# walaj/SeqLib

Hardware: AMD Instinct MI355X
Metric: aligned reads/sec (150 bp) via BWAAligner (higher is better)
Workload: dtype int32

## Files before the change

seqlib_amd/csrc/dev_chain.h:

```cpp
#pragma once
#include "dev_fm.h"
#include "dev_sort.h"
#include "dev_types.h"
#include "dev_pack.h"
#include "dev_kbtree.h"

__device__ __forceinline__ int next_slot(unsigned int *queue, int per_wave = 0)
{
    const int lane = threadIdx.x & 63;
    const unsigned int base = wave_take(queue, per_wave ? 1u : 64u);
    if (per_wave) return lane == 0 ? (int)base : 0x7fffffff;
    return (int)(base + lane);
}

struct ReadWS {
    int64_t *s_rbeg; qp_t *s_ql; int32_t *s_next; int32_t *s_score;
    int64_t *c_pos; int32_t *c_head, *c_tail, *c_n, *c_rid, *c_w, *c_first; int8_t *c_kept;
    int32_t *ia, *ib, *ic; uint64_t *srt;
    DReg *regs; DHit *hits;
    int cap;
    __device__ __forceinline__ int s_qbeg(int s) const { return QP_HI(s_ql[s]); }
    __device__ __forceinline__ int s_len(int s) const { return QP_LO(s_ql[s]); }
};

// ... 32 lines not shown
    for (int s = w.c_head[c]; s >= 0; s = w.s_next[s]) {
        const int qb = w.s_qbeg(s), l = w.s_len(s);
        if (qb >= end) wt += l;
        else if (qb + l > end) wt += (int)(qb + l - end);
        end = end > qb + l ? end : qb + l;
    }
    tmp = wt; wt = 0; end = 0;
    for (int s = w.c_head[c]; s >= 0; s = w.s_next[s]) {
        const int64_t rb = w.s_rbeg[s]; const int l = w.s_len(s);
        if (rb >= end) wt += l;
        else if (rb + l > end) wt += (int)(rb + l - end);
        end = end > rb + l ? end : rb + l;
    }
    wt = wt < tmp ? wt : tmp;
    return wt < 1 << 30 ? wt : (1 << 30) - 1;
}

template <typename I>
__device__ void dev_chain_read(const DevFM<I> &fm, const DevRef &R, const Chunk &ck, const slx_opt &opt, int r)
{
        ReadWS w = make_ws(ck, r);
        const int len = (int)(ck.offs[r + 1] - ck.offs[r]);
        const int n_intv = (int)ck.intv_n[r];
        const qp_t *iinfo = (const qp_t *)ck.intv_info + (size_t)r * ck.cap_intv;
        const I *ix0 = (const I *)ck.intv_x0 + (size_t)r * ck.cap_intv;
        const I *ix2 = (const I *)ck.intv_x2 + (size_t)r * ck.cap_intv;
        int ns = 0, nc = 0;
        int *ord = w.ia;
        KbTree kb;
        bool tree = false;
        int cc = -1, cc_tail = 0, cc_n = 0, cc_rid = 0;
        qp_t cc_fql = 0, cc_lql = 0;
        int64_t cc_frb = 0, cc_lrb = 0;
        for (int i = 0; i < n_intv; ++i) {
            const int qbeg = QP_HI(iinfo[i]), slen = QP_LO(iinfo[i]) - qbeg;
            const I x2 = ix2[i];
            const I step = x2 > (I)opt.max_occ ? x2 / (I)opt.max_occ : (I)1;
            I k = 0;
            for (int count = 0; k < x2 && count < opt.max_occ; k += step, ++count) {
                const int64_t rbeg = intv_pos<I>(fm, ix0[i], k);
                const int rid = dev_intv2rid(R, rbeg, rbeg + slen);
                if (rid < 0) continue;
                int lo = -1, lower_c = -1;
                bool to_add = true;
                if (nc) {
                    if (tree) lower_c = kb.lower(rbeg);
                    else {
                        int b = 0, e = nc;
                        while (b < e) { int m = (b + e) >> 1; if (w.c_pos[ord[m]] < rbeg) b = m + 1; else e = m; }
                        if (b == nc) lo = nc - 1;
                        else lo = rbeg < w.c_pos[ord[b]] ? b - 1 : b;
                        lower_c = lo >= 0 ? ord[lo] : -1;
                    }
                    if (lower_c >= 0) {
                        const int c = lower_c;
                        if (c != cc) {
                            const int first = w.c_head[c];
                            cc = c; cc_tail = w.c_tail[c]; cc_n = w.c_n[c]; cc_rid = w.c_rid[c];
                            cc_fql = w.s_ql[first]; cc_frb = w.s_rbeg[first];
                            cc_lql = w.s_ql[cc_tail]; cc_lrb = w.s_rbeg[cc_tail];
                        }
                        const int last = cc_tail;
                        const int l_qbeg = QP_HI(cc_lql), l_len = QP_LO(cc_lql);
                        const int64_t l_rbeg = cc_lrb;
                        const int64_t qend = l_qbeg + l_len, rend = l_rbeg + l_len;
                        int res;
                        if (rid != cc_rid) res = 0;
                        else if (qbeg >= QP_HI(cc_fql) && qbeg + slen <= qend && rbeg >= cc_frb && rbeg + slen <= rend) res = 1;
                        else if ((l_rbeg < R.l_pac || cc_frb < R.l_pac) && rbeg >= R.l_pac) res = 0;
                        else {
                            const int64_t x = qbeg - l_qbeg, y = rbeg - l_rbeg;
                            if (y >= 0 && x - y <= opt.w && y - x <= opt.w && x - l_len < opt.max_chain_gap && y - l_len < opt.max_chain_gap) {
                                const int s = ns++;
// ... 77 lines not shown
            int s_full = -1, cov = 0;
            bool same_diag = true;
            int64_t diag = 0;
            for (int s = w.c_head[c0]; s >= 0; s = w.s_next[s])
                if (w.s_qbeg(s) == 0 && w.s_len(s) == len) { s_full = s; diag = w.s_rbeg[s]; break; }
            if (s_full >= 0) {
                for (int s = w.c_head[c0]; s >= 0; s = w.s_next[s]) {
                    cov += w.s_len(s);
                    if (w.s_rbeg[s] - w.s_qbeg(s) != diag) same_diag = false;
                }
                if (same_diag) {
                    DReg g;
                    g.rb = diag; g.re = g.rb + len; g.qb = 0; g.qe = len; g.rid = w.c_rid[c0];
                    g.score = g.truesc = len * opt.a; g.sub = g.csub = g.sub_n = 0; g.w = opt.w; g.seedcov = cov; g.secondary = 0;
                    g.seedlen0 = len; g.n_comp = 0; g.frac_rep = ck.frac_rep[r]; g.hash = 0;
                    w.regs[0] = g;
                    ck.n_reg[r] = 1;
                    n_out = -1;
                }
            }
        }
        {
            int off = 0;
            for (int i = 0; i < n_out; ++i) {
                const int c = a[i];
                w.c_first[c] = off;
                for (int s = w.c_head[c]; s >= 0; s = w.s_next[s]) w.c_w[off++] = s;
            }
        }
        ck.n_chain[r] = n_out;
}

template <typename I>
__global__ void __launch_bounds__(128) k_chain(DevFM<I> fm, DevRef R, Chunk ck, DevOpt dopt, const int *order, unsigned int *queue, const unsigned int *n_slots, int per_wave)
{
    const slx_opt &opt = dopt.o;
    const int n_todo = (int)*n_slots;
    if (per_wave) __builtin_amdgcn_s_setprio(3);
    while (true) {
        const int slot = next_slot(queue, per_wave);
        if (__all(slot >= n_todo)) break;
        if (slot >= n_todo) continue;
        const int r = order ? order[slot] : slot;
        dev_chain_read<I>(fm, R, ck, opt, r);
    }
}
```

seqlib_amd/csrc/dev_fm.h:

```cpp
#pragma once
#include <hip/hip_runtime.h>
#include <stdint.h>

template <typename I>
struct DevFM {
    const uint32_t *bwt;
    const uint4 *occ;
    const uint64_t *sup;
    I primary;
    I L2[5];
    I seq_len;
    const I *sa_dense;
    const uint64_t *sa_samp;
    int sa_intv;
    const void *lut;
    int lut_k;
    int bwd_direct;
    const uint32_t *rep;
    uint64_t rep_mask;
    int rep_k;
};

__host__ __device__ __forceinline__ uint64_t rep_hash(uint64_t kmer)
{
    kmer ^= kmer >> 33; kmer *= 0xff51afd7ed558ccdull; kmer ^= kmer >> 33; kmer *= 0xc4ceb9fe1a85ec53ull; kmer ^= kmer >> 33;
    return kmer;
}

template <typename I>
struct alignas(2 * sizeof(I)) LutE { I lo, sz; };

template <typename I>
struct alignas(16) IntvE {
    I x0, x1, x2;
    uint32_t info;
};

template <typename I>
struct WorkLists {
    IntvE<I> *base;
    size_t stride;
    int cap;
    __device__ __forceinline__ IntvE<I> &at(int list, int e) { return base[((size_t)list * cap + e) * stride]; }
};

__device__ __forceinline__ void count_word(uint32_t w, int nb, uint32_t &c, uint32_t &g, uint32_t &t)
{
    uint32_t mask = nb >= 16 ? 0xffffffffu : (nb <= 0 ? 0u : ~(0xffffffffu >> (2 * nb)));
    w &= mask;
    uint32_t lo = w & 0x55555555u, hi = (w >> 1) & 0x55555555u;
    t += __popc(hi & lo);
    g += __popc(hi & ~lo);
    c += __popc(lo & ~hi);
// ... 98 lines not shown
```

seqlib_amd/csrc/dev_seed4.h:

```cpp
#pragma once
#include "dev_occ.h"
#include "dev_pack.h"

template <typename I>
struct RankLd {
    uint32_t c0, c1, c2, c3;
    uint32_t l0, l1, h0, h1;
    I s0, s1, s2, s3;
    uint32_t n;
};

template <typename I>
__device__ __forceinline__ void rank_issue(const DevFM<I> &fm, I pos, RankLd<I> &r)
{
    const I kk = pos - (pos >= fm.primary ? 1 : 0);
    const uint4 *blk = fm.occ + ((size_t)(kk >> 6) << 1);
    const uint4 cn = blk[0], pl = blk[1];
    r.c0 = cn.x; r.c1 = cn.y; r.c2 = cn.z; r.c3 = cn.w;
    r.l0 = pl.x; r.l1 = pl.y; r.h0 = pl.z; r.h1 = pl.w;
    r.n = ((uint32_t)kk & 63) + 1;
    if (sizeof(I) == 8) {
        const ulonglong2 *sp = (const ulonglong2 *)(fm.sup + ((uint64_t)kk >> 32) * 4);
        const ulonglong2 a = sp[0], b = sp[1];
        r.s0 = (I)a.x; r.s1 = (I)a.y; r.s2 = (I)b.x; r.s3 = (I)b.y;
    } else r.s0 = r.s1 = r.s2 = r.s3 = 0;
}

template <typename T>
__device__ __forceinline__ T sel4(int c, T v0, T v1, T v2, T v3) { const T lo = (c & 1) ? v1 : v0, hi = (c & 1) ? v3 : v2; return (c & 2) ? hi : lo; }

template <typename I, bool GT>
__device__ __forceinline__ void rank_finish(const RankLd<I> &r, int c, I &cnt_c, I &cnt_gt)
{
    const uint64_t m = ~0ull >> (64 - r.n);
    const uint32_t m0 = (uint32_t)m, m1 = (uint32_t)(m >> 32);
// ... 76 lines not shown
}

template <typename I>
__device__ __forceinline__ void fwd_step(const DevFM<I> &fm, I k0, I k1, I k2, int cq, I &o0, I &o1, I &o2)
{
    const int c = 3 - cq;
    RankLd<I> rk, rl;
    rank_issue<I>(fm, k1 - 1, rk); rank_issue<I>(fm, k1 - 1 + k2, rl);
    I ckc, ckg, clc, clg;
    rank_finish<I, true>(rk, c, ckc, ckg); rank_finish<I, true>(rl, c, clc, clg);
    o2 = clc - ckc;
    o1 = l2_of<I>(fm, c) + 1 + ckc;
    o0 = k0 + ((k1 <= fm.primary && k1 + k2 - 1 >= fm.primary) ? 1 : 0) + (clg - ckg);
}

template <typename I>
__global__ void k_kmer_lut(DevFM<I> fm, int K, LutE<I> *out)
{
    const uint64_t w = (uint64_t)blockIdx.x * blockDim.x + threadIdx.x;
    if (w >= (1ull << (2 * K))) return;
    I k0, k1, k2;
    set_intv4<I>(fm, (int)((w >> (2 * (K - 1))) & 3), k0, k1, k2);
    for (int t = 1; t < K; ++t) {
        I o0, o1, o2;
        fwd_step<I>(fm, k0, k1, k2, (int)((w >> (2 * (K - 1 - t))) & 3), o0, o1, o2);
        k0 = o0; k1 = o1; k2 = o2;
        if (k2 == 0) break;
    }
    LutE<I> e; e.lo = k2 ? k0 : (I)1; e.sz = k2;
    out[w] = e;
}

template <typename I>
__global__ void k_rep_filter(DevFM<I> fm, DevRef R, int kf, uint32_t *bits, uint64_t mask)
{
    const uint64_t n = (uint64_t)fm.seq_len;
    const uint64_t stride = (uint64_t)gridDim.x * blockDim.x;
    for (uint64_t i = (uint64_t)blockIdx.x * blockDim.x + threadIdx.x; i < n; i += stride) {
        const uint64_t p = (uint64_t)fm.sa_dense[i], q = (uint64_t)fm.sa_dense[i + 1];
        if (p + (uint64_t)kf > n || q + (uint64_t)kf > n) continue;
        RWin wp, wq; wp.bits = wq.bits = 0; wp.chunk = wq.chunk = -1;
        uint64_t kmer = 0;
        bool same = true;
        for (int t = 0; t < kf; ++t) {
            const int a = text_at(R, (int64_t)(p + t), wp), b = text_at(R, (int64_t)(q + t), wq);
            if (a != b) { same = false; break; }
            kmer = (kmer << 2) | (uint64_t)a;
        }
        if (!same) continue;
        const uint64_t h = rep_hash(kmer) & mask;
        atomicOr(bits + (h >> 5), 1u << (h & 31));
    }
}

template <typename I>
__global__ void __launch_bounds__(128) k_seed2_select(DevFM<I> fm, Chunk ck, DevOpt dopt, unsigned long long *p2mask, int *list, unsigned int *n_list,
                                                      uint32_t *items, unsigned int *n_items, uint32_t cap_items)
{
    const slx_opt &opt = dopt.o;
    const int t_ = blockIdx.x * blockDim.x + threadIdx.x;
    const int r = ck.spread > 1 ? t_ / ck.spread : t_;
    const bool live = r < ck.n_reads && (ck.spread <= 1 || t_ % ck.spread == 0);
    const int n = live ? (int)ck.intv_n[r] : 0;
    unsigned long long mask = 0;
    if (n > 0) {
        const uint64_t qoff = ck.offs[r];
        const int len = (int)(ck.offs[r + 1] - qoff);
        const int split_len = (int)(opt.min_seed_len * opt.split_factor + .499);
        QWin win; win.bits = 0; win.chunk = 0xffffffffu;
        auto qb = [&](int p) { return q_at(ck.codes, qoff + (uint64_t)p, win); };
        const bool use_rep = fm.rep != nullptr && fm.rep_k <= opt.min_seed_len && fm.rep_k > 0;
        const int kf = fm.rep_k;
        const uint64_t kmask = kf < 32 ? (1ull << (2 * kf)) - 1 : ~0ull;
        for (int k = 0; k < n; ++k) {
            const size_t o = (size_t)r * ck.cap_intv + k;
            const qp_t inf = ((const qp_t *)ck.intv_info)[o];
            const I s = ((const I *)ck.intv_x2)[o];
            const int start = QP_HI(inf), end = QP_LO(inf);
            if (end - start < split_len || s > (I)opt.split_width) continue;
            if (k >= 63) { mask |= 1ull << 63; break; }
            const int mid = (start + end) >> 1;
            if (qb(mid) > 3) continue;
            bool take = true;
            if (s == (I)1 && use_rep) {
                const int a_lo = mid - kf + 1 > 0 ? mid - kf + 1 : 0, a_hi = mid < len - kf ? mid : len - kf;
                uint64_t kmer = 0;
                int good = 0;
                for (int p = a_lo; p < a_lo + kf - 1; ++p) {
                    const int c = qb(p);
                    if (c > 3) { good = 0; kmer = 0; } else { kmer = ((kmer << 2) | (uint64_t)c) & kmask; ++good; }
                }
                take = false;
                for (int a = a_lo; a <= a_hi; ++a) {
                    const int c = qb(a + kf - 1);
                    if (c > 3) { good = 0; kmer = 0; continue; }
                    kmer = ((kmer << 2) | (uint64_t)c) & kmask; ++good;
                    if (good < kf) continue;
                    const uint64_t h = rep_hash(kmer) & fm.rep_mask;
                    if ((fm.rep[h >> 5] >> (h & 31)) & 1u) { take = true; break; }
                }
            }
            if (take) mask |= 1ull << k;
        }
    }
    if (live) p2mask[r] = mask;
    const uint32_t cnt = (uint32_t)__popcll(mask & ~(1ull << 63));
    const bool whole = (mask >> 63) != 0;
    uint32_t base = 0xffffffffu;
    {
        const uint32_t want = (live && !whole) ? cnt : 0u;
        uint32_t incl = want;
        for (int d = 1; d < 64; d <<= 1) { const uint32_t u = (uint32_t)__shfl_up((int)incl, d, 64); if ((int)(threadIdx.x & 63) >= d) incl += u; }
        const uint32_t total = (uint32_t)__shfl((int)incl, 63, 64);
        if (total) base = wave_take(n_items, total) + incl - want;
    }
    if (!live || !mask) return;
    if (!whole && cnt && base + cnt <= cap_items) {
        unsigned long long m = mask;
        for (uint32_t t = 0; t < cnt; ++t) { const int k = __ffsll((long long)m) - 1; m &= m - 1; items[base + t] = (uint32_t)r << 6 | (uint32_t)k; }
    } else {
        if (!whole) for (uint32_t t = 0; t < cnt && base + t < cap_items; ++t) items[base + t] = 0xffffffffu;
        list[wave_fetch_inc(n_list)] = r;
    }
}

template <typename QB>
__device__ __forceinline__ int kmer_codes(QB &qb, int p, int K, uint32_t &fw, uint32_t &rc)
{
    fw = 0; rc = 0;
    for (int t = 0; t < K; ++t) {
        const int c = qb(p + t);
        if (c > 3) return t;
// ... 782 lines not shown
```

seqlib_amd/csrc/slx_align.hip:

```cpp
#include <hip/hip_runtime.h>
#include <hipcub/hipcub.hpp>
#include <chrono>
#include <cmath>
#include <functional>
#include <unistd.h>
#include <cstdio>
#include <cstdlib>
#include <cstring>
#include <algorithm>
#include <mutex>
#include <string>
#include <thread>
#include <type_traits>
#include <vector>
#include "slx_internal.h"
#include "dev_seed4.h"
#include "dev_fin.h"
#include "dev_ext_wave.h"
#include "dev_ext_reg.h"
#include "dev_ext_lane.h"
#include "dev_ext_block.h"
#include "dev_ext_seg.h"
#include "dev_fin2.h"
#include "dev_chain_coop.h"
// ... 111 lines not shown
                           al->d_occ.as<uint4>(), n_blocks, sup);
        HIPCHK(hipGetLastError());
        HIPCHK(slx_wait_stream(al->stream));
        fm.occ = al->d_occ.as<uint4>();
        fm.sup = sup;
    }
    fm.primary = (I)idx->primary;
    for (int i = 0; i < 5; ++i) fm.L2[i] = (I)idx->L2[i];
    fm.seq_len = (I)idx->seq_len;
    if ((rc = build_lut<I>(al)) != SLX_OK) return rc;
    fm.sa_dense = nullptr;
    fm.sa_samp = al->d_sa_samp.as<uint64_t>();
    fm.sa_intv = idx->sa_intv;
    const uint64_t n1 = idx->seq_len + 1;
    al->have_dense = false;
    if ((rc = al->d_sa_dense.ensure(n1 * sizeof(I))) != SLX_OK) return rc;
    if (sizeof(I) == 4 && idx->dense_sa32.size() == n1) {
        HIPCHK(hipMemcpy(al->d_sa_dense.p, idx->dense_sa32.data(), n1 * 4, hipMemcpyHostToDevice));
    } else {
        const uint64_t n_sa = idx->sa.size();
        const int bs = 256;
        hipLaunchKernelGGL(k_sa_seed<I>, dim3((unsigned)((n_sa + bs - 1) / bs)), dim3(bs), 0, al->stream, fm, al->d_sa_dense.as<I>(), n_sa);
        hipLaunchKernelGGL(k_sa_walk<I>, dim3((unsigned)((n_sa + bs - 1) / bs)), dim3(bs), 0, al->stream, fm, al->d_sa_dense.as<I>(), n_sa);
        HIPCHK(hipGetLastError());
        HIPCHK(slx_wait_stream(al->stream));
    }
    al->have_dense = true;
    return SLX_OK;
}

template <typename I>
static int build_rep_filter(slx_aligner *al)
{
    al->rep_mask = 0;
    if (al->rep_k <= 0 || al->rep_k > 31 || !al->have_dense || al->host_idx->seq_len < 1024) return SLX_OK;
    uint64_t bits = 1ull << 20;
    while (bits < al->host_idx->seq_len * 8ull) bits <<= 1;
    while (al->d_rep.ensure(bits / 8) != SLX_OK) {
        (void)hipGetLastError();
        bits >>= 1;
        if (bits < al->host_idx->seq_len || bits < (1ull << 20)) { al->d_rep.release(); return SLX_OK; }
    }
    HIPCHK(hipMemsetAsync(al->d_rep.p, 0, bits / 8, al->stream));
    DevFM<I> fm = fm_of<I>(al);
    fm.sa_dense = al->d_sa_dense.as<I>();
    hipLaunchKernelGGL(k_rep_filter<I>, dim3(al->n_cu * 64), dim3(256), 0, al->stream, fm, al->ref, al->rep_k, al->d_rep.as<uint32_t>(), bits - 1);
    HIPCHK(hipGetLastError());
    HIPCHK(slx_wait_stream(al->stream));
    al->rep_mask = bits - 1;
    return SLX_OK;
}

#define SLX_MAX_WORKERS 8
static int env_hw_queues() { const char *e = getenv("GPU_MAX_HW_QUEUES"); const int v = e ? atoi(e) : 0; return v > 0 ? v : 4; }

static int default_workers()
{
    if (const char *e = getenv("SEQLIB_AMD_WORKERS")) { const int v = atoi(e); if (v >= 1 && v <= SLX_MAX_WORKERS) return v; }
    return 3;
}

static int make_worker_stream(slx_aligner *al, Worker *wk)
{
    if (al->stream_prio) {
        int least = 0, greatest = 0;
        HIPCHK(hipDeviceGetStreamPriorityRange(&least, &greatest));
        HIPCHK(hipStreamCreateWithPriority(&wk->stream, hipStreamNonBlocking, greatest));
    } else HIPCHK(hipStreamCreateWithFlags(&wk->stream, hipStreamNonBlocking));
    return SLX_OK;
}

static int set_seed_stream(slx_aligner *al, Worker *wk)
{
    if (wk->seed_stream) { HIPCHK(slx_wait_stream(wk->seed_stream)); HIPCHK(hipStreamDestroy(wk->seed_stream)); wk->seed_stream = nullptr; }
    if (al->seed_free_cus <= 0) return SLX_OK;
    const int words = (al->n_cu + 31) / 32;
    std::vector<uint32_t> mask((size_t)words, 0u);
    for (int cu = 0; cu < al->n_cu; ++cu)
        if ((cu & 31) < 32 - al->seed_free_cus) mask[(size_t)(cu >> 5)] |= 1u << (cu & 31);
    HIPCHK(hipExtStreamCreateWithCUMask(&wk->seed_stream, (uint32_t)words, mask.data()));
    if (!wk->ev_seed_in) HIPCHK(hipEventCreateWithFlags(&wk->ev_seed_in, hipEventDisableTiming));
    if (!wk->ev_seed_out) HIPCHK(hipEventCreateWithFlags(&wk->ev_seed_out, hipEventDisableTiming));
// ... 110 lines not shown
    slx_aligner *grp = new slx_aligner();
    grp->is_group = true;
    grp->subs.assign((size_t)n_dev, nullptr);
    grp->host_idx = idx;
    std::vector<int> rcs((size_t)n_dev, SLX_OK);
    std::vector<std::string> errs((size_t)n_dev);
    std::vector<std::thread> th;
    for (int i = 0; i < n_dev; ++i)
        th.emplace_back([&, i]() {
            rcs[(size_t)i] = create_one(idx, devices[i], false, &grp->subs[(size_t)i]);
            if (rcs[(size_t)i] != SLX_OK) errs[(size_t)i] = slx_last_error();
        });
    for (auto &t : th) t.join();
    for (int i = 0; i < n_dev; ++i)
        if (rcs[(size_t)i] != SLX_OK) {
            slx_set_error("device %d: %s", devices[i], errs[(size_t)i].c_str());
            const int rc = rcs[(size_t)i];
            slx_aligner_free(grp);
            return rc;
        }
    *out = grp;
    return SLX_OK;
}

extern "C" void slx_aligner_free(slx_aligner *al)
{
    if (!al) return;
    if (al->is_group) {
        for (slx_aligner *sub : al->subs) slx_aligner_free(sub);
        delete al;
        return;
    }
    (void)hipSetDevice(al->device);
    DevBuf *bufs[] = {&al->d_bwt, &al->d_occ, &al->d_sup, &al->d_lut, &al->d_rep, &al->d_sa_samp, &al->d_sa_dense, &al->d_pac, &al->d_ann_off, &al->d_ann_len, &al->d_ann_alt, &al->d_loglut, &al->o_hit_off,
                      &al->o_rid, &al->o_pos, &al->o_flag, &al->o_mapq, &al->o_score, &al->o_nm, &al->o_na, &al->o_ncig, &al->o_cig_off, &al->o_cigar, &al->o_xa, &al->o_sub,
                      &al->st_bases, &al->st_offs, &al->st_pack};
    for (DevBuf *b : bufs) b->release();
    for (Worker *wk : al->workers) {
        for (DevBuf *b : wk->all) b->release();
        for (int i = 0; i <= SLX_N_STAGES; ++i) if (wk->ev[i]) (void)hipEventDestroy(wk->ev[i]);
        for (int i = 0; i < 6; ++i) if (wk->dbg_ev[i]) (void)hipEventDestroy(wk->dbg_ev[i]);
        for (int i = 0; i < 6; ++i) if (wk->ev_probe[i]) (void)hipEventDestroy(wk->ev_probe[i]);
        if (wk->h_mail) (void)hipHostFree(wk->h_mail);
        if (wk->stream) (void)hipStreamDestroy(wk->stream);
        if (wk->seed_stream) (void)hipStreamDestroy(wk->seed_stream);
        if (wk->ev_seed_in) (void)hipEventDestroy(wk->ev_seed_in);
        if (wk->ev_seed_out) (void)hipEventDestroy(wk->ev_seed_out);
        delete wk;
    }
    if (al->h_bounce) (void)hipHostFree(al->h_bounce);
    if (al->stream) (void)hipStreamDestroy(al->stream);
    delete al;
    bool last;
    { std::lock_guard<std::mutex> g(g_live_mu); last = --g_live_aligners == 0; }
    if (last) pin_pool_release_all();
}

extern "C" int slx_aligner_set(slx_aligner *al, const char *key, int64_t value)
{
    if (!al || !key) return SLX_EINVAL;
    if (al->is_group) {
        std::lock_guard<std::mutex> call(al->call_mu);
        for (slx_aligner *sub : al->subs) { const int rc = slx_aligner_set(sub, key, value); if (rc != SLX_OK) return rc; }
        return SLX_OK;
    }
    std::lock_guard<std::mutex> call(al->call_mu);
    if (!strcmp(key, "chunk_reads")) { if (value < 1) return SLX_EINVAL; al->chunk_reads = value; }
// ... 39 lines not shown
    else if (!strcmp(key, "cig_fast_coop")) al->cig_fast_coop = value != 0;
    else if (!strcmp(key, "cig_lane_il")) al->cig_lane_il = value != 0;
    else if (!strcmp(key, "small_coop")) al->small_coop = value != 0;
    else if (!strcmp(key, "small_spread")) al->small_spread = value != 0;
    else if (!strcmp(key, "chain_sorted")) al->chain_sorted = value != 0;
    else if (!strcmp(key, "regs_sorted")) al->regs_sorted = value != 0;
    else if (!strcmp(key, "cand_top")) { if (value < 0) return SLX_EINVAL; al->cand_top = (int)value; }
    else if (!strcmp(key, "cand_rep_max")) { if (value < 0) return SLX_EINVAL; al->cand_rep_max = (int)value; }
    else if (!strcmp(key, "cand_rep")) { if (value < -1 || value > 101) return SLX_EINVAL; al->cand_rep = (int)value; }
    else if (!strcmp(key, "cand_lanes")) { if (value < -1 || value > 1) return SLX_EINVAL; al->cand_lanes = (int)value; }
    else if (!strcmp(key, "cig_lanes")) al->cig_lanes = value != 0;
    else if (!strcmp(key, "first_diag")) al->first_diag = value != 0;
    else if (!strcmp(key, "first_lanes")) al->first_lanes = value != 0;
    else if (!strcmp(key, "lane_narrow")) al->lane_narrow = value != 0;
    else if (!strcmp(key, "lane_pad")) al->lane_pad = (int)value;
    else if (!strcmp(key, "cand_lane_seeds")) { if (value < 1) return SLX_EINVAL; al->cand_lane_seeds = (int)value; }
    else if (!strcmp(key, "cand_cap")) { if (value < 1) return SLX_EINVAL; al->cand_cap = (int)value; }
    else if (!strcmp(key, "split_min")) al->split_min = (int)value;
    else if (!strcmp(key, "heavy_seeds")) { if (value < 1) return SLX_EINVAL; al->heavy_seeds = (int)value; }
    else if (!strcmp(key, "workers")) {
        if (value < 1 || value > SLX_MAX_WORKERS) return SLX_EINVAL;
        HIPCHK(hipSetDevice(al->device));
        while ((int)al->workers.size() < (int)value) { const int rc = add_worker(al); if (rc != SLX_OK) return rc; }
        al->n_workers = (int)value;
    }
    else if (!strcmp(key, "min_split")) { if (value < 1) return SLX_EINVAL; al->min_split = value; }
    else if (!strcmp(key, "seed_quota")) { if (value < 0 || value > (1 << 24)) return SLX_EINVAL; al->seed_quota = (int)value; }
    else if (!strcmp(key, "rep_k")) {
        if (value < 0 || value > 31) return SLX_EINVAL;
        al->rep_k = (int)value;
        HIPCHK(hipSetDevice(al->device));
        return al->wide ? build_rep_filter<uint64_t>(al) : build_rep_filter<uint32_t>(al);
    }
    else if (!strcmp(key, "top_heavy")) al->top_heavy = value != 0;
    else if (!strcmp(key, "top_reuse")) al->top_reuse = value != 0;
    else if (!strcmp(key, "p2_items")) al->p2_items = value != 0;
    else if (!strcmp(key, "p2_coop")) al->p2_coop = value != 0;
    else if (!strcmp(key, "p2_items_cap")) al->p2_items_cap = (int)value;
    else if (!strcmp(key, "seed_free_cus")) {
        if (value < 0 || value > 24) return SLX_EINVAL;
        HIPCHK(hipSetDevice(al->device));
        al->seed_free_cus = (int)value;
        for (Worker *wk : al->workers) { const int rc = set_seed_stream(al, wk); if (rc != SLX_OK) return rc; }
    }
    else if (!strcmp(key, "stream_prio")) {
        if (value < 0 || value > 1) return SLX_EINVAL;
        HIPCHK(hipSetDevice(al->device));
        al->stream_prio = (int)value;
        for (Worker *wk : al->workers) {
            HIPCHK(slx_wait_stream(wk->stream));
            HIPCHK(hipStreamDestroy(wk->stream));
            wk->stream = nullptr;
            const int rc = make_worker_stream(al, wk);
            if (rc != SLX_OK) return rc;
        }
    }
    else if (!strcmp(key, "threads")) { if (value < 64) return SLX_EINVAL; al->max_threads = (int)value; }
    else if (!strcmp(key, "zarena_bytes")) { if (value < 1024) return SLX_EINVAL; al->zcap = (unsigned long long)value; }
    else { slx_set_error("slx_aligner_set: unknown key %s", key); return SLX_EINVAL; }
    return SLX_OK;
}

extern "C" int slx_aligner_stage_ms(const slx_aligner *al, float ms[SLX_N_STAGES])
{
    if (!al || !ms) return SLX_EINVAL;
    if (al->is_group) {
        for (int i = 0; i < SLX_N_STAGES; ++i) { ms[i] = 0; for (const slx_aligner *sub : al->subs) ms[i] = std::max(ms[i], sub->stage_ms[i]); }
        return SLX_OK;
    }
    for (int i = 0; i < SLX_N_STAGES; ++i) ms[i] = al->stage_ms[i];
    return SLX_OK;
}

extern "C" int slx_aligner_probe_ms(const slx_aligner *al, float ms[SLX_N_PROBES], int64_t *n_reads)
{
    if (!al || !ms) return SLX_EINVAL;
    if (al->is_group) {
        int64_t n = 0;
        for (int i = 0; i < SLX_N_PROBES; ++i) ms[i] = 0;
        for (const slx_aligner *sub : al->subs) { for (int i = 0; i < SLX_N_PROBES; ++i) ms[i] += sub->probe_ms[i]; n += sub->probe_reads; }
        if (n_reads) *n_reads = n;
        return SLX_OK;
    }
    for (int i = 0; i < SLX_N_PROBES; ++i) ms[i] = al->probe_ms[i];
    if (n_reads) *n_reads = al->probe_reads;
    return SLX_OK;
}

extern "C" int64_t slx_aligner_counter(const slx_aligner *al, const char *key)
{
    if (!al || !key) return -1;
    if (!strcmp(key, "workers")) return al->is_group ? al->subs[0]->n_workers : al->n_workers;
    if (!strcmp(key, "hw_queues")) return al->hw_queues;
    if (!strcmp(key, "long_rounds") || !strcmp(key, "long_jobs")) {
        long long v = 0;
        const bool rounds = key[5] == 'r';
        auto take = [&](const slx_aligner *a) { for (const Worker *wk : a->workers) v = std::max(v, rounds ? (long long)wk->long_rounds_run : (long long)wk->long_jobs_run); };
        if (al->is_group) for (const slx_aligner *sub : al->subs) take(sub); else take(al);
        return v;
    }
    {
        if (!strcmp(key, "pseg_jobs")) {
            long long v = 0;
            auto take = [&](const slx_aligner *a) { for (const Worker *wk : a->workers) v += wk->pseg_stat; };
            if (al->is_group) for (const slx_aligner *sub : al->subs) take(sub); else take(al);
            return v;
        }
        if (!strcmp(key, "retries")) {
            long long v = 0;
            if (al->is_group) for (const slx_aligner *sub : al->subs) v += sub->n_retries; else v = al->n_retries;
            return v;
        }
        if (!strcmp(key, "regs_deferred") || !strcmp(key, "hits_wave_reads")) {
            long long v = 0;
            const int which = key[0] == 'h';
            auto take = [&](const slx_aligner *a) { for (const Worker *wk : a->workers) v += (long long)wk->fin_stat[which]; };
            if (al->is_group) for (const slx_aligner *sub : al->subs) take(sub); else take(al);
            return v;
        }
        static const char *const gs[3] = {"gseg_ok", "gseg_redo", "gseg_jobs"};
        for (int i = 0; i < 3; ++i)
            if (!strcmp(key, gs[i])) {
                long long v = 0;
                auto take = [&](const slx_aligner *a) { for (const Worker *wk : a->workers) v += wk->gseg_stat[i]; };
                if (al->is_group) for (const slx_aligner *sub : al->subs) take(sub); else take(al);
// ... 633 lines not shown
```

seqlib_amd/csrc/slx_align_types.h:

```cpp
#pragma once
#include <hip/hip_runtime.h>
#include <mutex>
#include <string>
#include <vector>
#include "slx_internal.h"
#include "dev_fm.h"
#include "dev_types.h"

#define HIPCHK(x)                                                                                   \
    do {                                                                                            \
        hipError_t e_ = (x);                                                                        \
        if (e_ != hipSuccess) {                                                                     \
            slx_set_error("HIP error %s at %s:%d (%s)", hipGetErrorString(e_), __FILE__, __LINE__, #x); \
            return e_ == hipErrorOutOfMemory ? SLX_ENOMEM : SLX_ENODEVICE;                          \
        }                                                                                           \
    } while (0)

struct DevBuf {
    void *p = nullptr;
    size_t cap = 0;
    int ensure(size_t bytes)
    {
        if (bytes <= cap) return SLX_OK;
        if (p) (void)hipFree(p);
// ... 67 lines not shown
    int id = 0;
    unsigned int max_seed_cnt = 0;
    hipEvent_t dbg_ev[6] = {nullptr, nullptr, nullptr, nullptr, nullptr, nullptr};
    DevBuf o_hit_off, o_rid, o_pos, o_flag, o_mapq, o_score, o_nm, o_na, o_ncig, o_cig_off, o_cigar, o_xa, o_sub;
    hipEvent_t ev[SLX_N_STAGES + 1];
    hipEvent_t ev_probe[6] = {nullptr, nullptr, nullptr, nullptr, nullptr, nullptr};
    float stage_ms[SLX_N_STAGES];
    float probe_ms[SLX_N_PROBES] = {0, 0, 0, 0, 0, 0};
    int n_chunks = 0;
    long long cnt[4] = {0, 0, 0, 0};
    int64_t n_hits = 0, n_cig = 0;
    int rc = SLX_OK;
    std::string err;
    std::vector<DevBuf *> all;
    void collect()
    {
        all = {&codes, &offs_rel, &intv_n, &intv_info, &intv_x0, &intv_x2, &l_rep, &seed_cnt, &seed_off, &scan_tmp, &s_rbeg, &s_ql, &s_next,
               &c_pos, &c_head, &c_tail, &c_n, &c_rid, &c_w, &c_first, &c_kept, &ia, &ib, &ic, &srt, &regs, &hits, &n_chain, &n_reg, &n_hit,
               &na, &frac_rep, &zarena, &cigpool, &counters, &lists, &hit_cnt, &cig_cnt, &hit_off_c, &cig_off_c, &order_key_in,
               &order_key_out, &order_in, &order_out, &queues, &sort_tmp, &jobs, &fast_list, &dp_list, &part_flag, &part_pos, &cand, &cand_base,
               &cand_cnt, &cand_off, &dbg_cyc, &order_tmp, &first_tab, &first_cnt, &first_off, &fb_list, &first_jobs, &len_stat, &s_score, &long_list, &long_scratch, &huge_rows, &p2mask, &p2list, &p2items, &p2long, &lane_jobs, &first_dp, &first_sorted, &first_bins, &cig_lane_list, &defer_list, &hits_big, &order_bin, &bin_cnt, &snap_ia, &snap_regs, &snap_nreg,
               &memo_idx, &memo_jobs, &memo_tab, &round_list, &todo_a, &todo_b, &spec_cnt, &seed3_buf, &job_key_in, &job_key_out, &job_val_in, &job_val_out, &job_sort_tmp, &pseg_jobs, &pseg_idx, &pseg_cnt, &gseg_jobs, &gseg_units, &gseg_wrec, &gseg_wout, &gseg_scratch, &gseg_cnt, &xseg_jobs, &xseg_state, &xseg_units, &xseg_out, &xseg_wrec, &xseg_wout, &xseg_scratch, &xseg_cnt,
               &o_hit_off, &o_rid, &o_pos, &o_flag, &o_mapq, &o_score, &o_nm, &o_na, &o_ncig, &o_cig_off, &o_cigar, &o_xa, &o_sub};
        for (auto &e : ev) e = nullptr;
    }
};

struct slx_aligner {
    std::vector<slx_aligner *> subs;
    bool is_group = false;
    int64_t merge_us = 0, call_us = 0;
    int device = 0;
    hipStream_t stream = nullptr;
    DevBuf d_bwt, d_occ, d_sup, d_lut, d_rep, d_sa_samp, d_sa_dense, d_pac, d_ann_off, d_ann_len, d_ann_alt, d_loglut;
    uint64_t rep_mask = 0;
    int rep_k = 19;
    bool wide = false;
    DevFM<uint32_t> fm32;
    DevFM<uint64_t> fm64;
    DevRef ref;
    bool dense_sa = true;
    bool have_dense = false;
    const slx_index *host_idx = nullptr;
    int64_t chunk_reads = 1 << 24;
    int cap_intv = 40;
    int cap_intv_long = 0;
    int long_predict = 0;
    int long_block = 32768;
    int long_seed3 = 1;
    int long_coop = 1;
    int bwd_direct = 0;
    int long_seg = 1;
    int xseg_wave_min = 2048;
    int xseg_fail = 0;
    int long_guess = 0;
    int long_budget = 1024;
    int regs_sorted = 0;
    int chain_sorted = 0;
    int small_spread = 1;
    int cig_fast_coop = 1;
    int cig_lane_il = 1;
    int hits_wave = 1;
    int small_coop = 1;
    int regs_defer = 1;
    int regs_big = 48;
    int coop_lim1 = 1 << 30, coop_lim2 = 1 << 30;
    int ext_split = 1;
    int heavy_sorted = 1;
    int cand_lanes = -1;
// ... 67 lines not shown
```

seqlib_amd/csrc/slx_chunk.inc:

```

__device__ __forceinline__ uint32_t nt4_of(uint32_t b)
{
    const uint32_t u = b & 0xDFu;
    const uint32_t x = (b >> 1) & 3u;
    const bool letter = u == 'A' || u == 'C' || u == 'G' || u == 'T';
    return b < 4u ? b : (letter ? (x ^ (x >> 1)) : 4u);
}

__global__ void k_encode(const uint8_t *ascii, uint8_t *codes, size_t n)
{
    const size_t n16 = (n + 15) >> 4;
    const size_t stride = (size_t)gridDim.x * blockDim.x;
    const bool aligned = ((uintptr_t)ascii & 3) == 0;
    for (size_t t = (size_t)blockIdx.x * blockDim.x + threadIdx.x; t < n16; t += stride) {
        const size_t i = t << 4;
        uint32_t w[4];
        if (aligned && i + 16 <= n) {
            const uint32_t *src = (const uint32_t *)(ascii + i);
#pragma unroll
            for (int k = 0; k < 4; ++k) w[k] = src[k];
        } else {
#pragma unroll
            for (int k = 0; k < 4; ++k) {
                w[k] = 0;
// ... 543 lines not shown
    ck.rng_state = rng_state;
    ck.cap_intv = caps.cap_intv;
    ck.intv_n = wk->intv_n.as<uint32_t>(); ck.intv_info = wk->intv_info.as<uint32_t>();
    ck.intv_x0 = wk->intv_x0.p; ck.intv_x2 = wk->intv_x2.p;
    ck.l_rep = wk->l_rep.as<int32_t>();
    ck.seed_off = wk->seed_off.as<uint64_t>();
    ck.n_chain = wk->n_chain.as<int32_t>(); ck.n_reg = wk->n_reg.as<int32_t>(); ck.n_hit = wk->n_hit.as<int32_t>();
    ck.na = wk->na.as<int32_t>(); ck.frac_rep = wk->frac_rep.as<float>();
    ck.zarena = wk->zarena.as<uint8_t>(); ck.zcap = caps.zcap; ck.zused = wk->counters.as<unsigned long long>();
    ck.cigpool = wk->cigpool.as<uint32_t>(); ck.cigcap = caps.cigcap; ck.cigused = wk->counters.as<unsigned long long>() + 1;
    ck.flags = (uint32_t *)(wk->counters.as<unsigned long long>() + 2);
    ck.log_lut = al->d_loglut.as<double>(); ck.log_lut_n = SLX_LOG_LUT_N;
    ck.lists = wk->lists.p; ck.cap_list = cap_list; ck.n_threads = n_threads;
    ck.hardclip = hardclip; ck.keepSecFrac = ksf; ck.maxSecondary = maxsec;
    ck.sam_mode = (opt->flag & SLX_F_REG2SAM) ? 1 : 0;
    ck.seed_cnt = wk->seed_cnt.as<unsigned long long>();
    const bool production = al->chain_mode == 1 && n >= al->split_min && !has_long;
    const bool use_cand = al->cand_mode == 1 && production;
    if (use_cand) {
        ENS(cand, (size_t)al->cand_cap * sizeof(DReg)); ENS(cand_base, (size_t)n * 4); ENS(cand_cnt, ((size_t)n + 2) * 8); ENS(cand_off, ((size_t)n + 2) * 8);
        HIPCHK(hipMemsetAsync(wk->cand_base.p, 0xff, (size_t)n * 4, st));
        ck.cand = wk->cand.as<DReg>(); ck.cand_base = wk->cand_base.as<int32_t>();
    }
    if (getenv("SLX_DEBUG_CYC")) {
        ENS(dbg_cyc, (size_t)n * 32);
        HIPCHK(hipMemsetAsync(wk->dbg_cyc.p, 0, (size_t)n * 32, st));
        ck.dbg_cyc = wk->dbg_cyc.as<unsigned long long>();
        ck.dbg_stage = atoi(getenv("SLX_DEBUG_CYC"));
    }
    DevOpt dopt; dopt.o = *opt;
    DevFM<I> fm = fm_of<I>(al);
    fm.sa_dense = (al->dense_sa && al->have_dense) ? al->d_sa_dense.as<I>() : nullptr;
    fm.rep = al->rep_mask ? al->d_rep.as<uint32_t>() : nullptr; fm.rep_mask = al->rep_mask; fm.rep_k = al->rep_k;
    fm.bwd_direct = (al->bwd_direct && fm.sa_dense && (sizeof(I) == 8 || (uint64_t)fm.seq_len < (1ULL << 31))) ? 1 : 0;

    (void)hipEventRecord(wk->ev[0], st);
    {
        const unsigned g = (unsigned)std::min<uint64_t>((n_bases / 16 + 255) / 256 + 1, 65535u * 4);
        hipLaunchKernelGGL(k_encode, dim3(g), dim3(256), 0, st, d_ascii + base0, wk->codes.as<uint8_t>(), (size_t)n_bases);
        hipLaunchKernelGGL(k_rel_offsets, dim3((unsigned)((n + 1 + 255) / 256)), dim3(256), 0, st, d_offs + r0, wk->offs_rel.as<uint64_t>(), n, base0);
    }
    (void)hipEventRecord(wk->ev[1], st);
    (void)hipEventRecord(wk->ev_probe[0], st);
    {
        hipStream_t ss = st;
        if (wk->seed_stream && production_seed(al, n, has_long)) {
            ss = wk->seed_stream;
            HIPCHK(hipEventRecord(wk->ev_seed_in, st));
            HIPCHK(hipStreamWaitEvent(ss, wk->ev_seed_in, 0));
        }
        unsigned int *qq = wk->queues.as<unsigned int>();
        hipLaunchKernelGGL((k_seed12m<I, 1>), dim3(seed_grid), dim3(bs), 0, ss, fm, al->ref, ck, dopt, qq + 29, seed_quota,
                           (const int *)nullptr, (const unsigned int *)nullptr, (const unsigned long long *)nullptr, (const uint32_t *)nullptr, (const unsigned int *)nullptr, 0u,
                           (uint32_t *)nullptr, (unsigned int *)nullptr, 0u);
        const uint32_t cap_items = (al->p2_items && n < (1 << 26)) ? (uint32_t)(al->p2_items_cap > 0 ? std::min(al->p2_items_cap, n) : n) : 0u;
        const uint32_t cap_long = (cap_items && al->p2_coop) ? cap_items : 0u;
        hipLaunchKernelGGL(k_seed2_select<I>, dim3((unsigned)(((int64_t)n * spread + bs - 1) / bs)), dim3(bs), 0, ss, fm, ck, dopt, wk->p2mask.as<unsigned long long>(), wk->p2list.as<int>(), qq + 35,
                           wk->p2items.as<uint32_t>(), qq + 37, cap_items);
        hipLaunchKernelGGL((k_seed12m<I, 2>), dim3(grid), dim3(bs), 0, ss, fm, al->ref, ck, dopt, qq + 36, 0u, wk->p2list.as<int>(), qq + 35,
                           wk->p2mask.as<unsigned long long>(), wk->p2items.as<uint32_t>(), qq + 37, cap_items, wk->p2long.as<uint32_t>(), qq + 38, cap_long);
        if (cap_long) hipLaunchKernelGGL(k_seed2_coop<I>, dim3((unsigned)(al->n_cu * 8)), dim3(64), 0, ss, fm, al->ref, ck, dopt, qq + 39, wk->p2long.as<uint32_t>(), qq + 38, cap_long);
        const int seed3_par = (max_len > 8192 && al->long_seed3) ? 4096 : 0x7fffffff;
        hipLaunchKernelGGL(k_seed3m<I>, dim3((unsigned)(((int64_t)n * spread + bs - 1) / bs)), dim3(bs), 0, ss, fm, al->ref, ck, dopt, seed3_par);
        if (seed3_par != 0x7fffffff) {
            ENS(seed3_buf, (size_t)n_bases * sizeof(Seed3Next<I>));
            hipLaunchKernelGGL(k_seed3_next<I>, dim3((unsigned)((n_bases + 255) / 256)), dim3(256), 0, ss, fm, al->ref, ck, dopt, seed3_par, (uint64_t)n_bases, wk->seed3_buf.as<Seed3Next<I>>());
// ... 427 lines not shown
```

Baseline: 69.32 million.

## Add positional repeat bitmap and chain anchor position derivation, tune chain launch bounds

Adds an optional per-reference-position repeat bitmap, built alongside the hashed k-mer repeat filter, so seed filtering can test one bit at the seed's SA position instead of rehashing every k-mer window inside the seed. Adds an optional chain-anchor mode that derives the reference position of unique sub-seeds contained in the two longest unique seeds, avoiding SA lookups. Both are behind new options that default to off. The only change that is always active is a min-blocks hint on k_chain's launch bounds, which may constrain registers and cause spills.

```diff
diff --git a/seqlib_amd/csrc/dev_chain.h b/seqlib_amd/csrc/dev_chain.h
--- a/seqlib_amd/csrc/dev_chain.h
+++ b/seqlib_amd/csrc/dev_chain.h
@@ -88,13 +88,32 @@
         int cc = -1, cc_tail = 0, cc_n = 0, cc_rid = 0;
         qp_t cc_fql = 0, cc_lql = 0;
         int64_t cc_frb = 0, cc_lrb = 0;
+        qp_t a0q = 0, a1q = 0;
+        I a0T = (I)-1, a1T = (I)-1;
+        if (fm.chain_anchor && n_intv > 1) {
+            int a0i = -1, a1i = -1;
+            for (int i = 0; i < n_intv; ++i) {
+                if (ix2[i] != (I)1) continue;
+                const qp_t q = iinfo[i];
+                const int l = QP_LO(q) - QP_HI(q);
+                if (a0i < 0 || l > QP_LO(a0q) - QP_HI(a0q)) { a1q = a0q; a1i = a0i; a0q = q; a0i = i; }
+                else if (a1i < 0 || l > QP_LO(a1q) - QP_HI(a1q)) { a1q = q; a1i = i; }
+            }
+            if (a0i >= 0) a0T = (I)intv_pos<I>(fm, ix0[a0i], (I)0);
+            if (a1i >= 0) a1T = (I)intv_pos<I>(fm, ix0[a1i], (I)0);
+        }
         for (int i = 0; i < n_intv; ++i) {
             const int qbeg = QP_HI(iinfo[i]), slen = QP_LO(iinfo[i]) - qbeg;
             const I x2 = ix2[i];
             const I step = x2 > (I)opt.max_occ ? x2 / (I)opt.max_occ : (I)1;
+            int64_t derived = -1;
+            if (x2 == (I)1) {
+                if (a0T != (I)-1 && qbeg >= QP_HI(a0q) && qbeg + slen <= QP_LO(a0q)) derived = (int64_t)a0T + (qbeg - QP_HI(a0q));
+                else if (a1T != (I)-1 && qbeg >= QP_HI(a1q) && qbeg + slen <= QP_LO(a1q)) derived = (int64_t)a1T + (qbeg - QP_HI(a1q));
+            }
             I k = 0;
             for (int count = 0; k < x2 && count < opt.max_occ; k += step, ++count) {
-                const int64_t rbeg = intv_pos<I>(fm, ix0[i], k);
+                const int64_t rbeg = derived >= 0 ? derived : intv_pos<I>(fm, ix0[i], k);
                 const int rid = dev_intv2rid(R, rbeg, rbeg + slen);
                 if (rid < 0) continue;
                 int lo = -1, lower_c = -1;
@@ -238,7 +257,7 @@
 }
 
 template <typename I>
-__global__ void __launch_bounds__(128) k_chain(DevFM<I> fm, DevRef R, Chunk ck, DevOpt dopt, const int *order, unsigned int *queue, const unsigned int *n_slots, int per_wave)
+__global__ void __launch_bounds__(128, (sizeof(I) == 8 ? 3 : 4)) k_chain(DevFM<I> fm, DevRef R, Chunk ck, DevOpt dopt, const int *order, unsigned int *queue, const unsigned int *n_slots, int per_wave)
 {
     const slx_opt &opt = dopt.o;
     const int n_todo = (int)*n_slots;
diff --git a/seqlib_amd/csrc/dev_fm.h b/seqlib_amd/csrc/dev_fm.h
--- a/seqlib_amd/csrc/dev_fm.h
+++ b/seqlib_amd/csrc/dev_fm.h
@@ -19,6 +19,9 @@
     const uint32_t *rep;
     uint64_t rep_mask;
     int rep_k;
+    const uint32_t *rep_pos;
+    int rep_pos_shift;
+    int chain_anchor;
 };
 
 __host__ __device__ __forceinline__ uint64_t rep_hash(uint64_t kmer)
diff --git a/seqlib_amd/csrc/dev_rep_pos.h b/seqlib_amd/csrc/dev_rep_pos.h
--- /dev/null
+++ b/seqlib_amd/csrc/dev_rep_pos.h
@@ -0,0 +1,25 @@
+#pragma once
+#include <stdint.h>
+#if defined(__HIPCC__)
+#define REP_POS_FN __host__ __device__ __forceinline__
+#else
+#define REP_POS_FN static inline
+#endif
+
+REP_POS_FN uint64_t rep_pos_words(uint64_t n, int shift) { return (((n - 1) >> shift) >> 5) + 2; }
+
+REP_POS_FN void rep_pos_span(uint64_t p, int k, int shift, uint64_t &w0, uint32_t &m0, uint32_t &m1)
+{
+    const uint64_t b0 = p >> shift, b1 = (p + (uint64_t)k - 1) >> shift;
+    w0 = b0 >> 5;
+    const int lo = (int)(b0 & 31), cnt = (int)(b1 - b0) + 1;
+    const uint64_t span = ((cnt >= 32 ? 0xffffffffull : (1ull << cnt) - 1ull)) << lo;
+    m0 = (uint32_t)span;
+    m1 = (uint32_t)(span >> 32);
+}
+
+REP_POS_FN bool rep_pos_test(const uint32_t *bits, uint64_t t, int shift)
+{
+    const uint64_t b = t >> shift;
+    return (bits[b >> 5] >> (b & 31)) & 1u;
+}
diff --git a/seqlib_amd/csrc/dev_seed4.h b/seqlib_amd/csrc/dev_seed4.h
--- a/seqlib_amd/csrc/dev_seed4.h
+++ b/seqlib_amd/csrc/dev_seed4.h
@@ -1,6 +1,7 @@
 #pragma once
 #include "dev_occ.h"
 #include "dev_pack.h"
+#include "dev_rep_pos.h"
 
 template <typename I>
 struct RankLd {
@@ -143,7 +144,7 @@
 }
 
 template <typename I>
-__global__ void k_rep_filter(DevFM<I> fm, DevRef R, int kf, uint32_t *bits, uint64_t mask)
+__global__ void k_rep_filter(DevFM<I> fm, DevRef R, int kf, uint32_t *bits, uint64_t mask, uint32_t *pos_bits, int pos_shift)
 {
     const uint64_t n = (uint64_t)fm.seq_len;
     const uint64_t stride = (uint64_t)gridDim.x * blockDim.x;
@@ -161,6 +162,14 @@
         if (!same) continue;
         const uint64_t h = rep_hash(kmer) & mask;
         atomicOr(bits + (h >> 5), 1u << (h & 31));
+        if (pos_bits) {
+            for (int e = 0; e < 2; ++e) {
+                uint64_t w0; uint32_t m0, m1;
+                rep_pos_span(e ? q : p, kf, pos_shift, w0, m0, m1);
+                if (m0 & ~pos_bits[w0]) atomicOr(pos_bits + w0, m0);
+                if (m1 & ~pos_bits[w0 + 1]) atomicOr(pos_bits + w0 + 1, m1);
+            }
+        }
     }
 }
 
@@ -182,6 +191,7 @@
         auto qb = [&](int p) { return q_at(ck.codes, qoff + (uint64_t)p, win); };
         const bool use_rep = fm.rep != nullptr && fm.rep_k <= opt.min_seed_len && fm.rep_k > 0;
         const int kf = fm.rep_k;
+        const bool use_pos = use_rep && fm.rep_pos != nullptr && fm.sa_dense != nullptr;
         const uint64_t kmask = kf < 32 ? (1ull << (2 * kf)) - 1 : ~0ull;
         for (int k = 0; k < n; ++k) {
             const size_t o = (size_t)r * ck.cap_intv + k;
@@ -195,20 +205,31 @@
             bool take = true;
             if (s == (I)1 && use_rep) {
                 const int a_lo = mid - kf + 1 > 0 ? mid - kf + 1 : 0, a_hi = mid < len - kf ? mid : len - kf;
-                uint64_t kmer = 0;
-                int good = 0;
-                for (int p = a_lo; p < a_lo + kf - 1; ++p) {
-                    const int c = qb(p);
-                    if (c > 3) { good = 0; kmer = 0; } else { kmer = ((kmer << 2) | (uint64_t)c) & kmask; ++good; }
-                }
                 take = false;
-                for (int a = a_lo; a <= a_hi; ++a) {
-                    const int c = qb(a + kf - 1);
-                    if (c > 3) { good = 0; kmer = 0; continue; }
-                    kmer = ((kmer << 2) | (uint64_t)c) & kmask; ++good;
-                    if (good < kf) continue;
-                    const uint64_t h = rep_hash(kmer) & fm.rep_mask;
-                    if ((fm.rep[h >> 5] >> (h & 31)) & 1u) { take = true; break; }
+                if (use_pos) {
+                    const int64_t T = intv_pos<I>(fm, ((const I *)ck.intv_x0)[o], (I)0);
+                    take = rep_pos_test(fm.rep_pos, (uint64_t)(T + (mid - start)), fm.rep_pos_shift);
+                }
+                const int in_lo = start > a_lo ? start : a_lo, in_hi = end - kf < a_hi ? end - kf : a_hi;
+                const bool inside = use_pos && in_lo <= in_hi;
+                for (int side = 0; side < 2 && !take; ++side) {
+                    const int lo = side == 0 ? a_lo : (inside ? in_hi + 1 : a_hi + 1);
+                    const int hi = side == 0 ? (inside ? in_lo - 1 : a_hi) : a_hi;
+                    if (lo > hi) continue;
+                    uint64_t kmer = 0;
+                    int good = 0;
+                    for (int p = lo; p < lo + kf - 1; ++p) {
+                        const int c = qb(p);
+                        if (c > 3) { good = 0; kmer = 0; } else { kmer = ((kmer << 2) | (uint64_t)c) & kmask; ++good; }
+                    }
+                    for (int a = lo; a <= hi; ++a) {
+                        const int c = qb(a + kf - 1);
+                        if (c > 3) { good = 0; kmer = 0; continue; }
+                        kmer = ((kmer << 2) | (uint64_t)c) & kmask; ++good;
+                        if (good < kf) continue;
+                        const uint64_t h = rep_hash(kmer) & fm.rep_mask;
+                        if ((fm.rep[h >> 5] >> (h & 31)) & 1u) { take = true; break; }
+                    }
                 }
             }
             if (take) mask |= 1ull << k;
diff --git a/seqlib_amd/csrc/slx_align.hip b/seqlib_amd/csrc/slx_align.hip
--- a/seqlib_amd/csrc/slx_align.hip
+++ b/seqlib_amd/csrc/slx_align.hip
@@ -167,22 +167,33 @@
 template <typename I>
 static int build_rep_filter(slx_aligner *al)
 {
-    al->rep_mask = 0;
-    if (al->rep_k <= 0 || al->rep_k > 31 || !al->have_dense || al->host_idx->seq_len < 1024) return SLX_OK;
+    al->rep_mask = 0; al->rep_pos_shift = -1; al->rep_bytes = 0;
+    if (al->rep_k <= 0 || al->rep_k > 31 || !al->have_dense || al->host_idx->seq_len < 1024) { al->d_rep.release(); al->d_rep_pos.release(); return SLX_OK; }
+    const uint64_t n = al->host_idx->seq_len;
+    const uint64_t per_sym = al->rep_pos ? 1ull : 8ull;
     uint64_t bits = 1ull << 20;
-    while (bits < al->host_idx->seq_len * 8ull) bits <<= 1;
+    while (bits < n * per_sym) bits <<= 1;
     while (al->d_rep.ensure(bits / 8) != SLX_OK) {
         (void)hipGetLastError();
         bits >>= 1;
-        if (bits < al->host_idx->seq_len || bits < (1ull << 20)) { al->d_rep.release(); return SLX_OK; }
-    }
+        if (bits < n * per_sym / 8 || bits < (1ull << 20)) { al->d_rep.release(); al->d_rep_pos.release(); return SLX_OK; }
+    }
+    int shift = -1;
+    if (al->rep_pos) {
+        for (shift = 0; shift <= 3 && al->d_rep_pos.ensure(rep_pos_words(n, shift) * 4) != SLX_OK; ++shift) (void)hipGetLastError();
+        if (shift > 3) { shift = -1; al->d_rep_pos.release(); }
+    } else al->d_rep_pos.release();
     HIPCHK(hipMemsetAsync(al->d_rep.p, 0, bits / 8, al->stream));
+    if (shift >= 0) HIPCHK(hipMemsetAsync(al->d_rep_pos.p, 0, rep_pos_words(n, shift) * 4, al->stream));
     DevFM<I> fm = fm_of<I>(al);
     fm.sa_dense = al->d_sa_dense.as<I>();
-    hipLaunchKernelGGL(k_rep_filter<I>, dim3(al->n_cu * 64), dim3(256), 0, al->stream, fm, al->ref, al->rep_k, al->d_rep.as<uint32_t>(), bits - 1);
+    hipLaunchKernelGGL(k_rep_filter<I>, dim3(al->n_cu * 64), dim3(256), 0, al->stream, fm, al->ref, al->rep_k, al->d_rep.as<uint32_t>(), bits - 1,
+                       shift >= 0 ? al->d_rep_pos.as<uint32_t>() : (uint32_t *)nullptr, shift >= 0 ? shift : 0);
     HIPCHK(hipGetLastError());
     HIPCHK(slx_wait_stream(al->stream));
     al->rep_mask = bits - 1;
+    al->rep_pos_shift = shift;
+    al->rep_bytes = bits / 8 + (shift >= 0 ? rep_pos_words(n, shift) * 4 : 0);
     return SLX_OK;
 }
 
@@ -359,7 +370,7 @@
         return;
     }
     (void)hipSetDevice(al->device);
-    DevBuf *bufs[] = {&al->d_bwt, &al->d_occ, &al->d_sup, &al->d_lut, &al->d_rep, &al->d_sa_samp, &al->d_sa_dense, &al->d_pac, &al->d_ann_off, &al->d_ann_len, &al->d_ann_alt, &al->d_loglut, &al->o_hit_off,
+    DevBuf *bufs[] = {&al->d_bwt, &al->d_occ, &al->d_sup, &al->d_lut, &al->d_rep, &al->d_rep_pos, &al->d_sa_samp, &al->d_sa_dense, &al->d_pac, &al->d_ann_off, &al->d_ann_len, &al->d_ann_alt, &al->d_loglut, &al->o_hit_off,
                       &al->o_rid, &al->o_pos, &al->o_flag, &al->o_mapq, &al->o_score, &al->o_nm, &al->o_na, &al->o_ncig, &al->o_cig_off, &al->o_cigar, &al->o_xa, &al->o_sub,
                       &al->st_bases, &al->st_offs, &al->st_pack};
     for (DevBuf *b : bufs) b->release();
@@ -465,6 +476,13 @@
         HIPCHK(hipSetDevice(al->device));
         return al->wide ? build_rep_filter<uint64_t>(al) : build_rep_filter<uint32_t>(al);
     }
+    else if (!strcmp(key, "rep_pos")) {
+        if (value < 0 || value > 1) return SLX_EINVAL;
+        al->rep_pos = (int)value;
+        HIPCHK(hipSetDevice(al->device));
+        return al->wide ? build_rep_filter<uint64_t>(al) : build_rep_filter<uint32_t>(al);
+    }
+    else if (!strcmp(key, "chain_anchor")) al->chain_anchor = value != 0;
     else if (!strcmp(key, "top_heavy")) al->top_heavy = value != 0;
     else if (!strcmp(key, "top_reuse")) al->top_reuse = value != 0;
     else if (!strcmp(key, "p2_items")) al->p2_items = value != 0;
@@ -524,6 +542,7 @@
 {
     if (!al || !key) return -1;
     if (!strcmp(key, "workers")) return al->is_group ? al->subs[0]->n_workers : al->n_workers;
+    if (!strcmp(key, "rep_bytes")) return (int64_t)(al->is_group ? al->subs[0]->rep_bytes : al->rep_bytes);
     if (!strcmp(key, "hw_queues")) return al->hw_queues;
     if (!strcmp(key, "long_rounds") || !strcmp(key, "long_jobs")) {
         long long v = 0;
diff --git a/seqlib_amd/csrc/slx_align_types.h b/seqlib_amd/csrc/slx_align_types.h
--- a/seqlib_amd/csrc/slx_align_types.h
+++ b/seqlib_amd/csrc/slx_align_types.h
@@ -123,9 +123,13 @@
     int64_t merge_us = 0, call_us = 0;
     int device = 0;
     hipStream_t stream = nullptr;
-    DevBuf d_bwt, d_occ, d_sup, d_lut, d_rep, d_sa_samp, d_sa_dense, d_pac, d_ann_off, d_ann_len, d_ann_alt, d_loglut;
+    DevBuf d_bwt, d_occ, d_sup, d_lut, d_rep, d_rep_pos, d_sa_samp, d_sa_dense, d_pac, d_ann_off, d_ann_len, d_ann_alt, d_loglut;
     uint64_t rep_mask = 0;
     int rep_k = 19;
+    int rep_pos = 0;
+    int rep_pos_shift = -1;
+    uint64_t rep_bytes = 0;
+    int chain_anchor = 0;
     bool wide = false;
     DevFM<uint32_t> fm32;
     DevFM<uint64_t> fm64;
diff --git a/seqlib_amd/csrc/slx_chunk.inc b/seqlib_amd/csrc/slx_chunk.inc
--- a/seqlib_amd/csrc/slx_chunk.inc
+++ b/seqlib_amd/csrc/slx_chunk.inc
@@ -599,6 +599,8 @@
     DevFM<I> fm = fm_of<I>(al);
     fm.sa_dense = (al->dense_sa && al->have_dense) ? al->d_sa_dense.as<I>() : nullptr;
     fm.rep = al->rep_mask ? al->d_rep.as<uint32_t>() : nullptr; fm.rep_mask = al->rep_mask; fm.rep_k = al->rep_k;
+    fm.rep_pos = (fm.rep && al->rep_pos_shift >= 0) ? al->d_rep_pos.as<uint32_t>() : nullptr; fm.rep_pos_shift = al->rep_pos_shift >= 0 ? al->rep_pos_shift : 0;
+    fm.chain_anchor = al->chain_anchor;
     fm.bwd_direct = (al->bwd_direct && fm.sa_dense && (sizeof(I) == 8 || (uint64_t)fm.seq_len < (1ULL << 31))) ? 1 : 0;
 
     (void)hipEventRecord(wk->ev[0], st);
```

Result: slower. 68.47 million (-1.2%).
